# bfGraph/STGraph

Hardware: NVIDIA B200
Metric: gcn_fused_aggregation_fwd_bwd_algorithmic_hbm_gbs (higher is better)
Workload: dtype f32

## Files before the change

include/stgraph_b200.h:

```cpp
#ifndef STGRAPH_B200_H_
#define STGRAPH_B200_H_

#include <stddef.h>
#include <stdint.h>

#ifdef __cplusplus
extern "C" {
#endif

#define STG_ABI_VERSION 3

typedef enum StgStatus {
  STG_OK = 0,
  STG_ERR_INVALID_ARGUMENT = -1,
  STG_ERR_CUDA = -2,
  STG_ERR_UNSUPPORTED = -3,
  STG_ERR_WORKSPACE_TOO_SMALL = -4,
  STG_ERR_CAPACITY = -5
} StgStatus;

typedef struct StgCsrView {
  const int32_t* row_offset;
  const int32_t* column_indices;
  const int32_t* eids;
  const int32_t* node_ids;
  int32_t num_nodes;
  int32_t num_edges;
  int32_t eid_base;
  int32_t eids_identity;
  const int32_t* hub_rows;
  const int32_t* hub_count;
  int32_t hub_threshold;
  int32_t hub_capacity;
// ... 2 lines not shown

int stg_abi_version(void);
const char* stg_last_error(void);
int stg_device_info(int device, int32_t* sm_count, int64_t* l2_bytes, int32_t* cc_major, int32_t* cc_minor);

int stg_agg_scaled_sum_f32(const StgCsrView* g, const float* x, int32_t feat,
                           const float* nbr_scale, const float* edge_scale,
                           const float* row_scale, float* out, void* stream);

typedef struct StgEdgeMeta {
  int32_t col;
  float scale;
} StgEdgeMeta;

int stg_csr_pack_edge_meta_f32(const StgCsrView* g, const float* nbr_scale, const float* edge_scale,
                               StgEdgeMeta* meta, void* stream);

int stg_agg_packed_sum_f32(const StgCsrView* g, const StgEdgeMeta* meta, const float* x, int32_t feat,
                           const float* row_scale, float* out, int32_t accumulate, void* stream);

int stg_agg_packed_sum_strided_f32(const StgCsrView* g, const StgEdgeMeta* meta, const float* x, int32_t feat,
                                   int32_t x_ld, const float* row_scale, float* out, int32_t out_ld,
                                   int32_t accumulate, void* stream);

int stg_agg_scaled_sum_accum_f32(const StgCsrView* g, const float* x, int32_t feat, const float* nbr_scale,
                                 const float* edge_scale, const float* row_scale, float* out, void* stream);

int stg_agg_scaled_sum_red_f32(const StgCsrView* g, const float* x, int32_t feat, const float* nbr_scale,
                               const float* edge_scale, const float* row_scale, float* out, void* stream);

int stg_agg_scaled_sum_rows_f32(const StgCsrView* g, const int32_t* out_rows, const float* x, int32_t feat,
                                const float* nbr_scale, const float* edge_scale, const float* row_scale, float* out,
                                int32_t accumulate, void* stream);

int stg_agg_packed_sum_rows_f32(const StgCsrView* g, const StgEdgeMeta* meta, const int32_t* out_rows, const float* x,
                                int32_t feat, const float* row_scale, float* out, int32_t accumulate, void* stream);

#define STG_MAX_PARTS 16
int stg_agg_scaled_sum_parts_f32(const StgCsrView* g, const float* const* x_parts, const int32_t* part_bounds,
                                 int32_t num_parts, int32_t feat, const float* nbr_scale, const float* edge_scale,
                                 const float* row_scale, float* out, void* stream);

int stg_halo_pull_f32(const float* const* x_parts, const int32_t* part_bounds, int32_t num_parts, const int64_t* ids,
                      int64_t n_ids, int32_t feat, float* out, int32_t max_blocks, void* stream);

int stg_halo_push_f32(const float* own, int32_t feat, const int64_t* send_rows, const int32_t* send_peer,
// ... 147 lines not shown
```

stgraph_b200/_lib.py:

```python
from __future__ import annotations

import ctypes
import os
import subprocess
from ctypes import POINTER, Structure, c_char_p, c_float, c_int32, c_int64, c_size_t, c_void_p

_HERE = os.path.dirname(os.path.abspath(__file__))
LIB_PATH = os.environ.get("STG_B200_LIB") or os.path.join(_HERE, "lib", "libstgraph_b200.so")
CSRC_DIR = os.path.join(_HERE, "csrc")

ABI_VERSION = 3
VM_MAX_TENSORS = 24
VM_MAX_INSTR = 96
VM_MAX_REGS = 48
VM_MAX_ACC = 8


class StgCsrView(Structure):

    _fields_ = [
        ("row_offset", c_void_p),
        ("column_indices", c_void_p),
        ("eids", c_void_p),
        ("node_ids", c_void_p),
        ("num_nodes", c_int32),
        ("num_edges", c_int32),
        ("eid_base", c_int32),
        ("eids_identity", c_int32),
        ("hub_rows", c_void_p),
        ("hub_count", c_void_p),
        ("hub_threshold", c_int32),
        ("hub_capacity", c_int32),
        ("work_queue", c_void_p),
    ]


class StgVmTensor(Structure):
    _fields_ = [("side", c_int32), ("bc0", c_int32), ("bc1", c_int32), ("pad", c_int32)]


class StgVmInstr(Structure):
    _fields_ = [
        ("op", ctypes.c_int16),
        ("phase", ctypes.c_int16),
        ("dst", ctypes.c_int16),
        ("a", ctypes.c_int16),
        ("b", ctypes.c_int16),
        ("pad", ctypes.c_int16),
        ("imm", c_float),
    ]


class StgVmProgram(Structure):
    _fields_ = [
        ("dim0", c_int32),
        ("dim1", c_int32),
        ("n_tensors", c_int32),
        ("n_instr", c_int32),
        ("n_regs", c_int32),
        ("n_acc", c_int32),
        ("n_pre", c_int32),
        ("n_loop", c_int32),
        ("acc_init", c_float * VM_MAX_ACC),
        ("acc_kind", c_int32 * VM_MAX_ACC),
        ("tensors", StgVmTensor * VM_MAX_TENSORS),
        ("instr", StgVmInstr * VM_MAX_INSTR),
    ]


_P = POINTER
_SIGNATURES = {
    "stg_abi_version": (ctypes.c_int, [], False),
    "stg_last_error": (c_char_p, [], False),
    "stg_device_info": (ctypes.c_int, [ctypes.c_int, _P(c_int32), _P(c_int64), _P(c_int32), _P(c_int32)], True),
    "stg_agg_scaled_sum_f32": (ctypes.c_int, [_P(StgCsrView), c_void_p, c_int32, c_void_p, c_void_p, c_void_p,
                                              c_void_p, c_void_p], True),
    "stg_agg_scaled_sum_accum_f32": (ctypes.c_int, [_P(StgCsrView), c_void_p, c_int32, c_void_p, c_void_p, c_void_p,
                                                    c_void_p, c_void_p], True),
    "stg_agg_scaled_sum_red_f32": (ctypes.c_int, [_P(StgCsrView), c_void_p, c_int32, c_void_p, c_void_p, c_void_p,
                                                  c_void_p, c_void_p], True),
    "stg_agg_scaled_sum_rows_f32": (ctypes.c_int, [_P(StgCsrView), c_void_p, c_void_p, c_int32, c_void_p, c_void_p, c_void_p,
                                                   c_void_p, c_int32, c_void_p], True),
    "stg_csr_pack_edge_meta_f32": (ctypes.c_int, [_P(StgCsrView), c_void_p, c_void_p, c_void_p, c_void_p], True),
    "stg_agg_packed_sum_f32": (ctypes.c_int, [_P(StgCsrView), c_void_p, c_void_p, c_int32, c_void_p, c_void_p, c_int32,
                                              c_void_p], True),
    "stg_agg_packed_sum_strided_f32": (ctypes.c_int, [_P(StgCsrView), c_void_p, c_void_p, c_int32, c_int32, c_void_p,
                                                      c_void_p, c_int32, c_int32, c_void_p], True),
    "stg_halo_push_f32": (ctypes.c_int, [c_void_p, c_int32, c_void_p, c_void_p, c_void_p, c_int64, _P(c_void_p), c_int32,
                                         c_int32, c_void_p], True),
    "stg_agg_packed_sum_rows_f32": (ctypes.c_int, [_P(StgCsrView), c_void_p, c_void_p, c_void_p, c_int32, c_void_p,
                                                   c_void_p, c_int32, c_void_p], True),
    "stg_rows_gather_f32": (ctypes.c_int, [c_void_p, c_int32, c_void_p, c_int64, c_void_p, c_int32, c_void_p], True),
    "stg_halo_send_f32": (ctypes.c_int, [c_void_p, c_int32, c_int32, c_int32, _P(c_int64), _P(c_void_p), c_void_p], True),
    "stg_halo_exchange_f32": (ctypes.c_int, [c_void_p, c_int32, c_void_p, _P(c_int64), c_void_p, _P(c_void_p), _P(c_void_p),
                                              c_void_p, c_int32, c_int32, c_int32, c_int32, c_void_p], True),
    "stg_peer_signal": (ctypes.c_int, [_P(c_void_p), c_int32, c_int32, c_int32, c_void_p], True),
    "stg_peer_wait": (ctypes.c_int, [c_void_p, c_int32, c_int32, c_int32, c_int64, c_void_p, c_void_p], True),
    "stg_agg_scaled_sum_parts_f32": (ctypes.c_int, [_P(StgCsrView), _P(c_void_p), _P(c_int32), c_int32, c_int32, c_void_p,
                                                    c_void_p, c_void_p, c_void_p, c_void_p], True),
    "stg_halo_pull_f32": (ctypes.c_int, [_P(c_void_p), _P(c_int32), c_int32, c_void_p, c_int64, c_int32, c_void_p, c_int32,
                                         c_void_p], True),
    "stg_agg_scaled_sum_f32_host": (ctypes.c_int, [_P(StgCsrView), c_void_p, c_int32, c_void_p, c_void_p, c_void_p,
                                                   c_void_p, c_void_p, c_size_t, c_void_p], True),
    "stg_agg_scaled_sum_f32_host_async": (ctypes.c_int, [_P(StgCsrView), c_void_p, c_int32, c_void_p, c_void_p, c_void_p,
                                                         c_void_p, c_void_p, c_size_t, c_void_p], True),
# ... 91 lines not shown
```

stgraph_b200/csrc/agg.cu:

```cuda
#include "common.cuh"

#include <cooperative_groups.h>

#include <algorithm>
#include <cstdlib>

namespace stg {
namespace {

constexpr int kBlockThreads = 256;
constexpr int kHubThreads = 512;

template <int VEC>
__device__ __forceinline__ typename VecT<VEC>::type ld_row(const float* p) {
  using T = typename VecT<VEC>::type;
  return __ldg(reinterpret_cast<const T*>(p));
}
template <int VEC>
__device__ __forceinline__ void st_row(float* p, typename VecT<VEC>::type v) {
  using T = typename VecT<VEC>::type;
  __stcs(reinterpret_cast<T*>(p), v);
}

struct AggParams {
  const int32_t* __restrict__ row_off;
  const int32_t* __restrict__ col;
  const int32_t* __restrict__ eids;
  const int32_t* __restrict__ hub_rows;
  const int32_t* __restrict__ hub_count;
  const int32_t* __restrict__ out_rows;
  const int2* __restrict__ meta;
  int* queue;
  int num_rows;
  int num_edges;
  int eid_base;
  int eids_identity;
  int hub_threshold;
  int hub_capacity;
  const float* __restrict__ x;
  float* __restrict__ out;
  int ld;
  int ld_out;
  int width;
  const float* __restrict__ ns;
  const float* __restrict__ es;
  const float* __restrict__ rs;
  int accumulate;
  int nparts;
  int bounds[STG_MAX_PARTS + 1];
  const float* xs[STG_MAX_PARTS];
};

__device__ __forceinline__ void red_add(float* p, float v) { atomicAdd(p, v); }
__device__ __forceinline__ void red_add(float* p, float2 v) { atomicAdd(reinterpret_cast<float2*>(p), v); }
__device__ __forceinline__ void red_add(float* p, float4 v) { atomicAdd(reinterpret_cast<float4*>(p), v); }

__device__ __forceinline__ const float* src_row(const AggParams& p, int c) {
  int o = 0;
#pragma unroll
  for (int q = 1; q < STG_MAX_PARTS; ++q) o += (q < p.nparts && c >= p.bounds[q]) ? 1 : 0;
  return p.xs[o] + static_cast<size_t>(c - p.bounds[o]) * p.ld;
}

enum AggMode { kPlain = 0, kParts = 1, kPacked = 2 };

template <int MODE>
__device__ __forceinline__ void load_col(const AggParams& p, int base, int end, int gl, int& c, float& ms) {
  c = 0;
  ms = 0.f;
  const int e = base + gl;
  if (e < end) {
    if constexpr (MODE == kPacked) {
      const int2 m = __ldcs(p.meta + e);
// ... 278 lines not shown
}

template <int VEC, int GROUP, int NACC>
__device__ __forceinline__ void write_row(const AggParams& p, int row, int gl, bool nonempty, float r,
                                          typename VecT<VEC>::type (&acc)[NACC]) {
  typename VecT<VEC>::type none[NACC];
#pragma unroll
  for (int k = 0; k < NACC; ++k) zero_vec(none[k]);
  write_row<VEC, GROUP, NACC>(p, row, gl, nonempty, r, acc, false, none);
}

template <int VEC, int GROUP, int NACC>
__device__ __forceinline__ void prefetch_row(const AggParams& p, int row, int gl, typename VecT<VEC>::type (&old)[NACC]) {
  using T = typename VecT<VEC>::type;
  const float* dst = p.out + static_cast<size_t>(row) * p.ld_out;
#pragma unroll
  for (int k = 0; k < NACC; ++k) {
    const int o = (gl + k * GROUP) * VEC;
    zero_vec(old[k]);
    if (o < p.width) old[k] = *reinterpret_cast<const T*>(dst + o);
  }
}

template <int VEC, int GROUP, int NACC, int MINB, int UNROLL, int MODE, bool PAIR = false, bool GQ = false>
__global__ void __launch_bounds__(kBlockThreads, MINB) agg_rows_pipe_kernel(const AggParams p, int slots_per_block) {
  using T = typename VecT<VEC>::type;
  constexpr int GPW = 32 / GROUP;
  __shared__ int next_slot;
  const int lane = threadIdx.x & 31;
  const int gl = lane & (GROUP - 1);
  const int gidx = lane / GROUP;
  const unsigned gmask = (GROUP == 32) ? 0xffffffffu : (((1u << GROUP) - 1u) << (lane & ~(GROUP - 1)));
  const int total_slots = (p.num_rows + GPW - 1) / GPW;
  const int first = GQ ? 0 : blockIdx.x * slots_per_block;
  const int last = GQ ? total_slots : min(first + slots_per_block, total_slots);
  int q_cur = 0, q_pos = slots_per_block, q_nxt = 0;
  if constexpr (GQ) {
    if (lane == 0) q_nxt = atomicAdd(p.queue, 1);
  } else {
    if (threadIdx.x == 0) next_slot = first;
    __syncthreads();
  }

  auto draw = [&]() {
    if constexpr (GQ) {
      if (q_pos == slots_per_block && q_cur < total_slots) {
        q_cur = __shfl_sync(0xffffffffu, q_nxt, 0) * slots_per_block;
        q_pos = 0;
        if (lane == 0 && q_cur < total_slots) q_nxt = atomicAdd(p.queue, 1);
      }
      return q_cur + q_pos++;
    } else {
      int s = 0;
      if (lane == 0) s = atomicAdd(&next_slot, 1);
      return __shfl_sync(0xffffffffu, s, 0);
    }
  };
  auto finish = [&]() {
    if constexpr (GQ) {
      __syncthreads();
      if (threadIdx.x == 0 && atomicAdd(p.queue + 1, 1) == static_cast<int>(gridDim.x) - 1) {
        p.queue[0] = 0;
        p.queue[1] = 0;
        __threadfence();
      }
    }
    grid_dependency_wait();
  };
  auto stage_a = [&](int slot, int& row, int& beg, int& end) {
    row = slot * GPW + gidx;
    if (slot >= last || row >= p.num_rows) { row = 0; beg = 0; end = -1; return; }
    beg = __ldg(p.row_off + row);
    end = __ldg(p.row_off + row + 1);
    if (p.out_rows) row = __ldg(p.out_rows + row);
  };
  auto drop_hub = [&](int& beg, int& end) {
    if (p.hub_threshold > 0 && (end - beg) > p.hub_threshold) beg = 0, end = -1;
  };

  int slot0, row0, beg0, end0, c0;
  int row1, beg1, end1, c1;
  int row2, beg2, end2;
  float s0, r0, m0, m1;
  slot0 = draw();
  if (slot0 >= last) { finish(); return; }
  stage_a(slot0, row0, beg0, end0);
  int slot1 = draw();
  stage_a(slot1, row1, beg1, end1);
  int slot2 = draw();
  stage_a(slot2, row2, beg2, end2);
  drop_hub(beg0, end0);
  load_col<MODE>(p, beg0, end0, gl, c0, m0);
  drop_hub(beg1, end1);
  load_col<MODE>(p, beg1, end1, gl, c1, m1);
  load_scale<MODE>(p, beg0, end0, gl, c0, m0, s0);
  r0 = (end0 >= 0 && p.rs) ? __ldg(p.rs + row0) : 1.f;

  while (slot0 < last) {
    const int slot3 = draw();
    int row3, beg3, end3;
    stage_a(slot3, row3, beg3, end3);
    drop_hub(beg2, end2);
    int c2;
    float m2;
    load_col<MODE>(p, beg2, end2, gl, c2, m2);
    float s1;
    load_scale<MODE>(p, beg1, end1, gl, c1, m1, s1);
    const float r1 = (end1 >= 0 && p.rs) ? __ldg(p.rs + row1) : 1.f;

    if (end0 >= 0) {
      T acc[NACC];
      T old[NACC];
      const bool rmw = NACC <= 2 && p.accumulate == 1;
      if constexpr (NACC <= 2) {
        if (rmw) prefetch_row<VEC, GROUP, NACC>(p, row0, gl, old);
      }
      if constexpr (PAIR) {
        static_assert(VEC == 4 && GROUP == 32 && NACC == 1, "pair form: one row per warp, float4 lanes");
        accumulate_edges_pair<UNROLL, MODE>(p, beg0, end0, lane, acc[0], c0, 0.f, s0);
      } else {
#pragma unroll
        for (int k = 0; k < NACC; ++k) zero_vec(acc[k]);
        accumulate_edges<VEC, GROUP, NACC, UNROLL, MODE>(p, beg0, end0, 0, 1, gl, gmask, acc, c0, s0);
      }
      write_row<VEC, GROUP, NACC>(p, row0, gl, end0 > beg0, r0, acc, rmw, old);
    }
    slot0 = slot1; row0 = row1; beg0 = beg1; end0 = end1; c0 = c1; s0 = s1; r0 = r1;
    slot1 = slot2; row1 = row2; beg1 = beg2; end1 = end2; c1 = c2; m1 = m2;
    slot2 = slot3; row2 = row3; beg2 = beg3; end2 = end3;
  }
  finish();
}

template <int VEC, int GROUP, int NACC, int MODE, bool PAIR = false>
__global__ void __launch_bounds__(kBlockThreads) agg_rows_kernel(const AggParams p) {
  using T = typename VecT<VEC>::type;
  constexpr int GROUPS_PER_WARP = 32 / GROUP;
  const int lane = threadIdx.x & 31;
  const int gl = lane & (GROUP - 1);
  const unsigned gmask = (GROUP == 32) ? 0xffffffffu : (((1u << GROUP) - 1u) << (lane & ~(GROUP - 1)));
  const int warp = blockIdx.x * (kBlockThreads / 32) + (threadIdx.x >> 5);
  const int row = warp * GROUPS_PER_WARP + lane / GROUP;
  if (row >= p.num_rows) return;
  const int beg = __ldg(p.row_off + row);
  const int end = __ldg(p.row_off + row + 1);
  if (p.hub_threshold > 0 && (end - beg) > p.hub_threshold) return;

  T acc[NACC];
// ... 126 lines not shown
    return e == nullptr || e[0] != '0';
  }();
  return on;
}

inline int queue_chunk() {
  static const int v = [] {
    const char* e = getenv("STG_AGG_CHUNK");
    const int c = e ? atoi(e) : 4;
    return c < 0 ? 0 : (c > 4096 ? 4096 : c);
  }();
  return v;
}

inline int hub_grid_mult(int num_edges) {
  static const int v = [] {
    const char* e = getenv("STG_HUB_GRID");
    const int c = e ? atoi(e) : 0;
    return c < 0 ? 0 : (c > 4 ? 4 : c);
  }();
  return v > 0 ? v : (num_edges >= (1 << 24) ? 1 : 2);
}

template <int VEC, int GROUP, int NACC, int MODE>
int launch_agg(const AggParams& p, cudaStream_t stream) {
  constexpr int rows_per_block = (kBlockThreads / 32) * (32 / GROUP);
  const int blocks = (p.num_rows + rows_per_block - 1) / rows_per_block;
  const bool hubs = p.hub_threshold > 0 && p.hub_rows != nullptr;
  const bool overlap = hubs && p.num_edges >= (1 << 18);
  if (hubs) {
    agg_hub_kernel<VEC, GROUP, NACC, MODE><<<hub_grid_mult(p.num_edges) * (sm_count() / kHubCluster) * kHubCluster, kHubThreads, 0, stream>>>(p);
    STG_LAUNCH_CHECK("agg_hub_kernel");
  }
  if (blocks > 0) {
    const bool queue = p.num_rows >= 2 * sm_count() * 4 * (kBlockThreads / 32);
    bool launched = false;
    if constexpr (GROUP == 32 && MODE != kParts) if (queue) {
      launched = true;
      constexpr int MINB = 4;
      constexpr int kRowsPerWarp = 32;
      constexpr int slots_per_block = (kBlockThreads / 32) * kRowsPerWarp;
      const int pblocks = (p.num_rows + slots_per_block - 1) / slots_per_block;
      const bool gq = p.queue != nullptr && queue_chunk() > 0;
      const int gblocks = std::min(sm_count() * MINB, (p.num_rows + 7) / 8);
      if constexpr (VEC == 4 && NACC == 1) {
        if (p.width > 64 && pair_mode()) {
          if (gq) {
            STG_CUDA(launch_overlapped(agg_rows_pipe_kernel<VEC, GROUP, NACC, MINB, 8, MODE, true, true>, gblocks, kBlockThreads,
                                       stream, overlap, p, queue_chunk()));
          } else {
// ... 48 lines not shown
  return launch_agg<VEC, 32, 4, MODE>(p, stream);
}

__global__ void __launch_bounds__(256) pack_edge_meta_kernel(const AggParams p, int2* __restrict__ meta) {
  const int stride = gridDim.x * blockDim.x;
  for (int e = blockIdx.x * blockDim.x + threadIdx.x; e < p.num_edges; e += stride) {
    const int c = ld_stream(p.col + e);
    float sc = 1.f;
    if (p.ns) sc = __ldg(p.ns + c);
    if (p.es) {
      const int eid = p.eids_identity ? e : (ld_stream(p.eids + e) - p.eid_base);
      sc *= __ldg(p.es + eid);
    }
    __stcs(meta + e, make_int2(c, __float_as_int(sc)));
  }
}

}

int agg_scaled_sum_device(const StgCsrView* g, const float* x, int32_t feat, const float* ns,
                          const float* es, const float* rs, float* out, cudaStream_t stream,
                          int nparts = 0, const float* const* parts = nullptr, const int32_t* bounds = nullptr,
                          int accumulate = 0, const int32_t* out_rows = nullptr, const StgEdgeMeta* meta = nullptr,
                          int x_ld = 0, int out_ld = 0) {
  AggParams p;
  p.out_rows = out_rows;
  p.meta = reinterpret_cast<const int2*>(meta);
  p.queue = g->work_queue;
  p.accumulate = accumulate;
  p.nparts = nparts;
  for (int q = 0; q < STG_MAX_PARTS; ++q) p.xs[q] = q < nparts ? parts[q] : nullptr;
  for (int q = 0; q <= STG_MAX_PARTS; ++q) p.bounds[q] = (nparts > 0 && q <= nparts) ? bounds[q] : 0;
  p.row_off = g->row_offset;
  p.col = g->column_indices;
  p.eids = g->eids;
  p.hub_rows = g->hub_rows;
  p.hub_count = g->hub_count;
  p.num_rows = g->num_nodes;
  p.num_edges = g->num_edges;
  p.eid_base = g->eid_base;
  p.eids_identity = g->eids_identity;
  p.hub_threshold = (g->hub_rows && g->hub_count) ? g->hub_threshold : 0;
  p.hub_capacity = g->hub_capacity;
  p.ld = x_ld > 0 ? x_ld : feat;
  p.ld_out = out_ld > 0 ? out_ld : feat;
  p.ns = ns;
  p.es = es;
  p.rs = rs;
  bool al16 = aligned16(out), al8 = aligned8(out);
  if (nparts == 0) {
    al16 = al16 && aligned16(x);
    al8 = al8 && aligned8(x);
  }
  for (int q = 0; q < nparts; ++q) {
    al16 = al16 && aligned16(parts[q]);
    al8 = al8 && aligned8(parts[q]);
  }
  int vec = 1;
  if (feat % 4 == 0 && p.ld % 4 == 0 && p.ld_out % 4 == 0 && al16) vec = 4;
  else if (feat % 2 == 0 && p.ld % 2 == 0 && p.ld_out % 2 == 0 && al8) vec = 2;
  if (vec == 4 && feat > 32 && feat <= 64 && nparts == 0 && narrow_vec2() && g->work_queue != nullptr &&
      g->num_nodes >= 2 * sm_count() * 4 * (kBlockThreads / 32))
    vec = 2;
  const int chunk = 32 * 4 * vec;
  for (int f0 = 0; f0 < feat; f0 += chunk) {
    p.x = x ? x + f0 : nullptr;
    for (int q = 0; q < nparts; ++q) p.xs[q] = parts[q] + f0;
    p.out = out + f0;
    p.width = min(chunk, feat - f0);
    int rc;
    const int avg_degree = g->num_nodes > 0 ? g->num_edges / g->num_nodes : -1;
    if (nparts > 0) {
      if (vec == 4) rc = dispatch_group<4, kParts>(p, stream, avg_degree);
      else if (vec == 2) rc = dispatch_group<2, kParts>(p, stream, avg_degree);
      else rc = dispatch_group<1, kParts>(p, stream, avg_degree);
    } else if (meta != nullptr) {
      if (vec == 4) rc = dispatch_group<4, kPacked>(p, stream, avg_degree);
      else if (vec == 2) rc = dispatch_group<2, kPacked>(p, stream, avg_degree);
      else rc = dispatch_group<1, kPacked>(p, stream, avg_degree);
    } else {
      if (vec == 4) rc = dispatch_group<4, kPlain>(p, stream, avg_degree);
      else if (vec == 2) rc = dispatch_group<2, kPlain>(p, stream, avg_degree);
      else rc = dispatch_group<1, kPlain>(p, stream, avg_degree);
    }
    if (rc != STG_OK) return rc;
  }
  return STG_OK;
// ... 148 lines not shown
  const int blocks = static_cast<int>(std::min<int64_t>((static_cast<int64_t>(g->num_edges) + 255) / 256, 8 * sm_count()));
  pack_edge_meta_kernel<<<blocks, 256, 0, as_stream(stream)>>>(p, reinterpret_cast<int2*>(meta));
  STG_LAUNCH_CHECK("pack_edge_meta_kernel");
  return STG_OK;
}

STG_API int stg_agg_packed_sum_strided_f32(const StgCsrView* g, const StgEdgeMeta* meta, const float* x, int32_t feat,
                                           int32_t x_ld, const float* row_scale, float* out, int32_t out_ld,
                                           int32_t accumulate, void* stream) {
  int rc = validate_view(g, false);
  if (rc != STG_OK) return rc;
  STG_CHECK_ARG(feat > 0, "feat must be positive (got %d)", feat);
  STG_CHECK_ARG(x_ld >= feat && out_ld >= feat, "row strides (%d, %d) must be >= feat (%d)", x_ld, out_ld, feat);
  STG_CHECK_ARG(accumulate >= 0 && accumulate <= 2, "accumulate must be 0, 1 or 2 (got %d)", accumulate);
  if (g->num_nodes == 0) return STG_OK;
  STG_CHECK_ARG(g->num_edges == 0 || (meta != nullptr && aligned8(meta)),
                "meta must be a non-NULL, 8-byte aligned device pointer");
  STG_CHECK_ARG(x != nullptr && out != nullptr, "x / out is NULL");
  STG_CHECK_ARG(x != out, "x and out must not alias");
  return agg_scaled_sum_device(g, x, feat, nullptr, nullptr, row_scale, out, as_stream(stream), 0, nullptr, nullptr,
                               accumulate, nullptr, g->num_edges == 0 ? nullptr : meta, x_ld, out_ld);
}

STG_API int stg_agg_packed_sum_f32(const StgCsrView* g, const StgEdgeMeta* meta, const float* x, int32_t feat,
                                   const float* row_scale, float* out, int32_t accumulate, void* stream) {
  return stg_agg_packed_sum_strided_f32(g, meta, x, feat, feat, row_scale, out, feat, accumulate, stream);
}

STG_API int stg_agg_packed_sum_rows_f32(const StgCsrView* g, const StgEdgeMeta* meta, const int32_t* out_rows,
                                        const float* x, int32_t feat, const float* row_scale, float* out,
                                        int32_t accumulate, void* stream) {
  int rc = validate_view(g, false);
  if (rc != STG_OK) return rc;
  STG_CHECK_ARG(feat > 0, "feat must be positive (got %d)", feat);
  STG_CHECK_ARG(accumulate >= 0 && accumulate <= 2, "accumulate must be 0, 1 or 2 (got %d)", accumulate);
  if (g->num_nodes == 0) return STG_OK;
  STG_CHECK_ARG(g->num_edges == 0 || (meta != nullptr && aligned8(meta)),
                "meta must be a non-NULL, 8-byte aligned device pointer");
  STG_CHECK_ARG(x != nullptr && out != nullptr, "x / out is NULL");
  STG_CHECK_ARG(x != out, "x and out must not alias");
  return agg_scaled_sum_device(g, x, feat, nullptr, nullptr, row_scale, out, as_stream(stream), 0, nullptr, nullptr,
                               accumulate, out_rows, g->num_edges == 0 ? nullptr : meta);
}
```

stgraph_b200/graph/static/csr.py:

```python
from __future__ import annotations

import ctypes
import os

import numpy as np
import torch

from ... import _lib

HUB_THRESHOLD = int(os.environ.get("STG_HUB_THRESHOLD", "1024"))
PACK_META = os.environ.get("STG_PACK_META", "1") != "0"
MAX_META_REPACKS = 16


def _edges_to_device(edge_list, device, num_nodes=None):
    if isinstance(edge_list, tuple) and len(edge_list) == 2 and not np.isscalar(edge_list[0]) \
            and len(np.shape(edge_list[0])) == 1 and len(edge_list[0]) != 2:
        src, dst = edge_list
        src = torch.as_tensor(src)
        dst = torch.as_tensor(dst)
    else:
        if isinstance(edge_list, torch.Tensor):
            e = edge_list
        else:
            e = torch.from_numpy(np.asarray(edge_list, dtype=np.int64).reshape(-1, 2))
        e = e.reshape(-1, 2)
        src, dst = e[:, 0], e[:, 1]
    if src.is_floating_point() or dst.is_floating_point() or src.dtype == torch.bool:
        raise TypeError("vertex ids must be integers")
    src, dst = src.to(device=device), dst.to(device=device)
    if num_nodes is not None and src.numel() > 0:
        lo = int(torch.minimum(src.min(), dst.min()))
        hi = int(torch.maximum(src.max(), dst.max()))
        if lo < 0 or hi >= int(num_nodes):
# ... 72 lines not shown
            return None
        from ... import kernels

        meta = kernels.pack_edge_meta(self.view(), nbr_scale, edge_scale, device=self.row_offset.device)
        self._meta_cache = [(key, (nbr_scale, edge_scale), meta)] + self._meta_cache[:1]
        return meta

    def invalidate_packed_meta(self):
        if self._meta_misses > MAX_META_REPACKS:
            self.pack_enabled = bool(PACK_META)
        self._meta_cache = []
        self._meta_misses = 0

    def prepare_hub_schedule(self, sync: bool = True):
        n, e = self.num_nodes, self.num_edges
        cap = e // max(HUB_THRESHOLD, 1) + 1
        dev = self.row_offset.device
        self._hub_rows = torch.empty(cap, dtype=torch.int32, device=dev)
        self._hub_count = torch.zeros(1, dtype=torch.int32, device=dev)
        _lib.call("stg_csr_hub_rows", self.row_offset.data_ptr(), n, HUB_THRESHOLD, self._hub_rows.data_ptr(),
                  cap, self._hub_count.data_ptr(), _lib.current_stream_ptr())
        self._hub_enabled = True
        self._hub_sync = sync
        if sync:
            self._hub_enabled = int(self._hub_count.item()) > 0
        self._view = None
        self._alt_views = {}

    def view(self) -> _lib.StgCsrView:
        if self._view is None:
            v = _lib.StgCsrView()
            v.row_offset = self.row_offset.data_ptr()
            v.column_indices = self.column_indices.data_ptr()
            v.eids = self.eids.data_ptr() if self.eids is not None else None
            v.node_ids = self.node_ids.data_ptr() if self.node_ids is not None else None
            v.num_nodes = self.num_nodes
            v.num_edges = self.num_edges
            v.eid_base = self.eid_base
            v.eids_identity = 1 if self.eids_identity else 0
            if self._hub_enabled:
                v.hub_rows = self._hub_rows.data_ptr()
                v.hub_count = self._hub_count.data_ptr()
                v.hub_threshold = HUB_THRESHOLD
                v.hub_capacity = int(self._hub_rows.shape[0])
            else:
                v.hub_rows = None
                v.hub_count = None
                v.hub_threshold = 0
                v.hub_capacity = 0
            self._work_queue = torch.zeros(2, dtype=torch.int32, device=self.row_offset.device)
# ... 21 lines not shown
        enabled = True
        if getattr(self, "_hub_sync", False):
            cnt = min(int(count.item()), cap)
            enabled = cnt > 0
            if cnt > 1:
                r = rows[:cnt].long()
                length = (self.row_offset[r + 1] - self.row_offset[r]).long()
                order = torch.sort(length * self.num_nodes + (self.num_nodes - 1 - r), descending=True).indices
                rows[:cnt] = rows[:cnt][order]
        v = _lib.StgCsrView()
        for name, _ in _lib.StgCsrView._fields_:
            setattr(v, name, getattr(base, name))
        v.hub_rows = rows.data_ptr() if enabled else None
        v.hub_count = count.data_ptr() if enabled else None
        v.hub_threshold = threshold if enabled else 0
        v.hub_capacity = cap if enabled else 0
        alt[threshold] = (v, rows, count)
    return alt[threshold][0]


CSR.view_with_hub_threshold = _alt_view


def build_csr_pair(src: torch.Tensor, dst: torch.Tensor, num_nodes: int, want_perm: bool = False):
    assert src.is_cuda and dst.is_cuda, "stgraph_b200 builds graphs on the GPU only (no CPU fallback)"
    dev = src.device
    e = int(src.shape[0])
    n = int(num_nodes)
    i32 = dict(dtype=torch.int32, device=dev)
    f_ro = torch.empty(n + 1, **i32)
    f_col = torch.empty(e, **i32)
    f_eid = torch.empty(e, **i32)
    f_nid = torch.empty(n, **i32)
    b_ro = torch.empty(n + 1, **i32)
    b_col = torch.empty(e, **i32)
    b_eid = torch.empty(e, **i32)
    b_nid = torch.empty(n, **i32)
    in_deg = torch.empty(n, **i32)
    out_deg = torch.empty(n, **i32)
    perm = torch.empty(e, **i32) if want_perm else None
    n_unique = torch.zeros(1, **i32)
    ws_bytes = _lib.load().stg_csr_build_workspace_bytes(e, n)
    ws = torch.empty(ws_bytes, dtype=torch.uint8, device=dev)
    _lib.call("stg_csr_build", src.data_ptr(), dst.data_ptr(), e, n,
              f_ro.data_ptr(), f_col.data_ptr(), f_eid.data_ptr(), f_nid.data_ptr(),
              b_ro.data_ptr(), b_col.data_ptr(), b_eid.data_ptr(), b_nid.data_ptr(),
# ... 12 lines not shown
```

stgraph_b200/kernels.py:

```python
from __future__ import annotations

import ctypes

import torch

from . import _lib

launch_count = 0


def _check(t: torch.Tensor, name: str, dtype=torch.float32):
    if not isinstance(t, torch.Tensor):
        raise TypeError(f"{name} must be a torch.Tensor")
    if not t.is_cuda:
        raise RuntimeError(f"{name} must live on a CUDA device (stgraph_b200 has no CPU path)")
    if t.dtype != dtype:
        raise TypeError(f"{name} must be {dtype}, got {t.dtype}")
    if not t.is_contiguous():
        raise ValueError(f"{name} must be contiguous")
    return t


def agg_scaled_sum(view: _lib.StgCsrView, x: torch.Tensor, nbr_scale=None, edge_scale=None, row_scale=None,
                   out: torch.Tensor | None = None, accumulate=False, stream=None, out_rows=None) -> torch.Tensor:
    global launch_count
    _check(x, "x")
    n = view.num_nodes
    if out_rows is not None:
        _check(out_rows, "out_rows", torch.int32)
        if out is None or out_rows.numel() != n:
            raise ValueError("out_rows needs out= and one entry per view row")
        n = out.shape[0]
    if x.dim() < 2:
        raise ValueError("x must be [rows, feat...]")
    feat = x.numel() // max(x.shape[0], 1)
    for nm, t in (("nbr_scale", nbr_scale), ("edge_scale", edge_scale)):
        if t is not None:
            _check(t, nm)
    if nbr_scale is not None and nbr_scale.numel() != x.shape[0]:
        raise ValueError(f"nbr_scale must have one entry per row of x ({x.shape[0]}), got {nbr_scale.numel()}")
    if row_scale is not None:
        _check(row_scale, "row_scale")
        if row_scale.numel() != n:
            raise ValueError(f"row_scale must have {n} elements, got {row_scale.numel()}")
    if edge_scale is not None and edge_scale.numel() < view.num_edges:
        raise ValueError(f"edge_scale has {edge_scale.numel()} elements for {view.num_edges} edges")
    if out is None:
        if x.shape[0] != n:
            raise ValueError(f"x has {x.shape[0]} rows for a view of {n} rows: pass out= for a row slice")
        out = torch.empty_like(x)
    else:
        _check(out, "out")
        if out.shape[0] != n or out.numel() != n * feat:
            raise ValueError(f"out must be [{n}, {feat}], got {tuple(out.shape)}")
    if n == 0 or feat == 0 or view.num_nodes == 0:
        return out
    if out_rows is not None:
        _lib.call("stg_agg_scaled_sum_rows_f32", ctypes.byref(view), out_rows.data_ptr(), x.data_ptr(), feat,
                  _lib.ptr(nbr_scale), _lib.ptr(edge_scale), _lib.ptr(row_scale), out.data_ptr(),
                  {False: 0, True: 1, "red": 2}[accumulate], stream if stream is not None else _lib.current_stream_ptr())
        launch_count += 1 + (1 if view.hub_threshold > 0 else 0)
        return out
    fn = {False: "stg_agg_scaled_sum_f32", True: "stg_agg_scaled_sum_accum_f32", "red": "stg_agg_scaled_sum_red_f32"}[accumulate]
    _lib.call(fn, ctypes.byref(view), x.data_ptr(), feat, _lib.ptr(nbr_scale), _lib.ptr(edge_scale), _lib.ptr(row_scale),
              out.data_ptr(), stream if stream is not None else _lib.current_stream_ptr())
    launch_count += 1 + (1 if view.hub_threshold > 0 else 0)
    return out


def pack_edge_meta(view: _lib.StgCsrView, nbr_scale=None, edge_scale=None, out: torch.Tensor | None = None,
                   device=None) -> torch.Tensor:
    global launch_count
    for nm, t in (("nbr_scale", nbr_scale), ("edge_scale", edge_scale)):
        if t is not None:
            _check(t, nm)
    if edge_scale is not None and edge_scale.numel() < view.num_edges:
        raise ValueError(f"edge_scale has {edge_scale.numel()} elements for {view.num_edges} edges")
    if out is None:
        ref = nbr_scale if nbr_scale is not None else edge_scale
        dev = device if device is not None else (ref.device if ref is not None else torch.device("cuda", torch.cuda.current_device()))
        out = torch.empty(view.num_edges, 2, dtype=torch.int32, device=dev)
    else:
        _check(out, "out", torch.int32)
        if out.numel() != 2 * view.num_edges:
            raise ValueError(f"meta must be int32 [{view.num_edges}, 2]")
# ... 4 lines not shown
    launch_count += 1
    return out


def padded_rows(rows: int, feat: int, device, dtype=torch.float32) -> torch.Tensor:
    ld = (feat + 31) // 32 * 32
    return torch.empty(rows, ld, dtype=dtype, device=device)[:, :feat]


def _row_stride(t: torch.Tensor, name: str) -> int:
    if t.dim() == 2 and not t.is_contiguous():
        if not t.is_cuda:
            raise RuntimeError(f"{name} must live on a CUDA device (stgraph_b200 has no CPU path)")
        if t.dtype != torch.float32:
            raise TypeError(f"{name} must be torch.float32, got {t.dtype}")
        if t.shape[1] > 0 and (t.stride(1) != 1 or t.stride(0) < t.shape[1]):
            raise ValueError(f"{name} must have dense rows (stride(1) == 1, stride(0) >= feat)")
        return int(t.stride(0))
    _check(t, name)
    return t.numel() // max(t.shape[0], 1)


def agg_packed_sum(view: _lib.StgCsrView, meta: torch.Tensor, x: torch.Tensor, row_scale=None,
                   out: torch.Tensor | None = None, accumulate=False, stream=None) -> torch.Tensor:
    global launch_count
    x_ld = _row_stride(x, "x")
    _check(meta, "meta", torch.int32)
    n = view.num_nodes
    if meta.numel() < 2 * view.num_edges:
        raise ValueError(f"meta has {meta.numel() // 2} entries for {view.num_edges} edges")
    if x.dim() < 2:
        raise ValueError("x must be [rows, feat...]")
    feat = x.shape[1] if x.dim() == 2 else x.numel() // max(x.shape[0], 1)
    if row_scale is not None:
        _check(row_scale, "row_scale")
        if row_scale.numel() != n:
            raise ValueError(f"row_scale must have {n} elements, got {row_scale.numel()}")
    if out is None:
        if x.shape[0] != n:
            raise ValueError(f"x has {x.shape[0]} rows for a view of {n} rows: pass out= for a row slice")
        out = padded_rows(n, feat, x.device) if x_ld != feat else torch.empty_like(x)
    out_ld = _row_stride(out, "out")
    if out.shape[0] != n or out.numel() != n * feat:
        raise ValueError(f"out must be [{n}, {feat}], got {tuple(out.shape)}")
    if n == 0 or feat == 0:
        return out
    _lib.call("stg_agg_packed_sum_strided_f32", ctypes.byref(view), meta.data_ptr(), x.data_ptr(), feat, x_ld,
              _lib.ptr(row_scale), out.data_ptr(), out_ld, {False: 0, True: 1, "red": 2}[accumulate],
              stream if stream is not None else _lib.current_stream_ptr())
    launch_count += 1 + (1 if view.hub_threshold > 0 else 0)
    return out


def agg_packed_sum_rows(view: _lib.StgCsrView, meta: torch.Tensor, out_rows, x: torch.Tensor, row_scale, out: torch.Tensor,
                        accumulate=False, stream=None) -> torch.Tensor:
    global launch_count
    _check(x, "x")
    _check(out, "out")
    _check(meta, "meta", torch.int32)
    if meta.numel() < 2 * view.num_edges:
        raise ValueError(f"meta has {meta.numel() // 2} entries for {view.num_edges} edges")
    feat = x.numel() // max(x.shape[0], 1)
    if out.numel() != out.shape[0] * feat:
        raise ValueError(f"out must be [rows, {feat}], got {tuple(out.shape)}")
    if out_rows is not None:
        _check(out_rows, "out_rows", torch.int32)
        if out_rows.numel() != view.num_nodes:
            raise ValueError("out_rows needs one entry per view row")
    elif out.shape[0] != view.num_nodes:
        raise ValueError(f"out has {out.shape[0]} rows for a view of {view.num_nodes} rows")
    if row_scale is not None:
        _check(row_scale, "row_scale")
        if row_scale.numel() != out.shape[0]:
            raise ValueError(f"row_scale must have one entry per row of out ({out.shape[0]}), got {row_scale.numel()}")
    if view.num_nodes == 0 or feat == 0:
        return out
    _lib.call("stg_agg_packed_sum_rows_f32", ctypes.byref(view), meta.data_ptr(), _lib.ptr(out_rows), x.data_ptr(), feat,
              _lib.ptr(row_scale), out.data_ptr(), {False: 0, True: 1, "red": 2}[accumulate],
              stream if stream is not None else _lib.current_stream_ptr())
    launch_count += 1 + (1 if view.hub_threshold > 0 else 0)
    return out


def agg_scaled_sum_graph(csr, x: torch.Tensor, nbr_scale=None, edge_scale=None, row_scale=None,
                         out: torch.Tensor | None = None) -> torch.Tensor:
    meta = csr.packed_meta(nbr_scale, edge_scale) if getattr(csr, "pack_enabled", False) else None
    if meta is None:
        return agg_scaled_sum(csr.view(), x, nbr_scale, edge_scale, row_scale, out=out)
    return agg_packed_sum(csr.view(), meta, x, row_scale, out=out)


def gemm_tn(a: torch.Tensor, b: torch.Tensor, colsum: bool = False, out: torch.Tensor | None = None):
    global launch_count
    for nm, t in (("a", a), ("b", b)):
        if not t.is_cuda or t.dtype != torch.float32 or t.dim() != 2:
            raise TypeError(f"{nm} must be a 2-D float32 CUDA tensor")
        if t.shape[1] > 1 and t.stride(1) != 1:
            raise ValueError(f"{nm} must have unit stride along its rows (got strides {tuple(t.stride())})")
    if a.shape[0] != b.shape[0]:
        raise ValueError(f"a and b must have the same number of rows ({a.shape[0]} vs {b.shape[0]})")
    m, k, nc = a.shape[0], a.shape[1], b.shape[1]
    lda = a.stride(0) if m > 1 else max(k, 1)
    ldb = b.stride(0) if m > 1 else max(nc, 1)
    if out is not None and (out.shape != (k, nc) or not out.is_contiguous() or out.dtype != torch.float32):
        raise ValueError(f"out must be a contiguous float32 [{k}, {nc}] tensor")
    c = out if out is not None else torch.empty(k, nc, device=a.device, dtype=torch.float32)
    cs = torch.empty(nc, device=a.device, dtype=torch.float32) if colsum else None
    need = _lib.call("stg_gemm_tn_workspace_bytes", m, k, nc)
    ws = torch.empty(need // 4, device=a.device, dtype=torch.float32) if need else None
    _lib.call("stg_gemm_tn_f32", a.data_ptr(), lda, b.data_ptr(), ldb, m, k, nc, c.data_ptr(), _lib.ptr(cs), _lib.ptr(ws), need,
              _lib.current_stream_ptr())
    launch_count += 2 if need else 1
# ... 44 lines not shown
```

Before: 1003.

## Split hub rows into warp segments inside the persistent row-queue kernel

Adds a hub-segment schedule in which high-degree rows are split into 16 or 128 virtual slots interleaved with normal rows in one global work queue. Each warp accumulates its strided slice of edges into a partials buffer, and the last warp to finish, detected by an atomic counter, reduces the partials and writes the row. This folds the separate hub launch into a single kernel and balances load across warps. The cost is extra partial-buffer traffic, thread fences, and a host-side schedule built at graph setup.

Result: slower. 734.3, median of 6 (-26.8%).

```diff
diff --git a/include/stgraph_b200.h b/include/stgraph_b200.h
--- a/include/stgraph_b200.h
+++ b/include/stgraph_b200.h
@@ -8,7 +8,7 @@
 extern "C" {
 #endif
 
-#define STG_ABI_VERSION 3
+#define STG_ABI_VERSION 4
 
 typedef enum StgStatus {
   STG_OK = 0,
@@ -57,6 +57,23 @@
 int stg_agg_packed_sum_strided_f32(const StgCsrView* g, const StgEdgeMeta* meta, const float* x, int32_t feat,
                                    int32_t x_ld, const float* row_scale, float* out, int32_t out_ld,
                                    int32_t accumulate, void* stream);
+
+typedef struct StgHubSegments {
+  const int32_t* vslot;
+  const int32_t* segments;
+  int32_t* counters;
+  float* partials;
+  int64_t partial_capacity;
+  int32_t num_slots;
+  int32_t num_segments;
+} StgHubSegments;
+
+int stg_agg_scaled_sum_seg_f32(const StgCsrView* g, const StgHubSegments* seg, const float* x, int32_t feat,
+                               const float* nbr_scale, const float* edge_scale, const float* row_scale, float* out,
+                               void* stream);
+int stg_agg_packed_sum_seg_f32(const StgCsrView* g, const StgHubSegments* seg, const StgEdgeMeta* meta, const float* x,
+                               int32_t feat, int32_t x_ld, const float* row_scale, float* out, int32_t out_ld,
+                               void* stream);
 
 int stg_agg_scaled_sum_accum_f32(const StgCsrView* g, const float* x, int32_t feat, const float* nbr_scale,
                                  const float* edge_scale, const float* row_scale, float* out, void* stream);
diff --git a/stgraph_b200/_lib.py b/stgraph_b200/_lib.py
--- a/stgraph_b200/_lib.py
+++ b/stgraph_b200/_lib.py
@@ -9,7 +9,7 @@
 LIB_PATH = os.environ.get("STG_B200_LIB") or os.path.join(_HERE, "lib", "libstgraph_b200.so")
 CSRC_DIR = os.path.join(_HERE, "csrc")
 
-ABI_VERSION = 3
+ABI_VERSION = 4
 VM_MAX_TENSORS = 24
 VM_MAX_INSTR = 96
 VM_MAX_REGS = 48
@@ -35,6 +35,19 @@
     ]
 
 
+class StgHubSegments(Structure):
+
+    _fields_ = [
+        ("vslot", c_void_p),
+        ("segments", c_void_p),
+        ("counters", c_void_p),
+        ("partials", c_void_p),
+        ("partial_capacity", c_int64),
+        ("num_slots", c_int32),
+        ("num_segments", c_int32),
+    ]
+
+
 class StgVmTensor(Structure):
     _fields_ = [("side", c_int32), ("bc0", c_int32), ("bc1", c_int32), ("pad", c_int32)]
 
@@ -81,6 +94,10 @@
                                                   c_void_p, c_void_p], True),
     "stg_agg_scaled_sum_rows_f32": (ctypes.c_int, [_P(StgCsrView), c_void_p, c_void_p, c_int32, c_void_p, c_void_p, c_void_p,
                                                    c_void_p, c_int32, c_void_p], True),
+    "stg_agg_scaled_sum_seg_f32": (ctypes.c_int, [_P(StgCsrView), _P(StgHubSegments), c_void_p, c_int32, c_void_p, c_void_p,
+                                                  c_void_p, c_void_p, c_void_p], True),
+    "stg_agg_packed_sum_seg_f32": (ctypes.c_int, [_P(StgCsrView), _P(StgHubSegments), c_void_p, c_void_p, c_int32, c_int32,
+                                                  c_void_p, c_void_p, c_int32, c_void_p], True),
     "stg_csr_pack_edge_meta_f32": (ctypes.c_int, [_P(StgCsrView), c_void_p, c_void_p, c_void_p, c_void_p], True),
     "stg_agg_packed_sum_f32": (ctypes.c_int, [_P(StgCsrView), c_void_p, c_void_p, c_int32, c_void_p, c_void_p, c_int32,
                                               c_void_p], True),
diff --git a/stgraph_b200/csrc/agg.cu b/stgraph_b200/csrc/agg.cu
--- a/stgraph_b200/csrc/agg.cu
+++ b/stgraph_b200/csrc/agg.cu
@@ -10,6 +10,7 @@
 
 constexpr int kBlockThreads = 256;
 constexpr int kHubThreads = 512;
+constexpr int kHubWarps = kHubThreads / 32;
 
 template <int VEC>
 __device__ __forceinline__ typename VecT<VEC>::type ld_row(const float* p) {
@@ -49,6 +50,11 @@
   int nparts;
   int bounds[STG_MAX_PARTS + 1];
   const float* xs[STG_MAX_PARTS];
+  const int* __restrict__ vslot;
+  const int4* __restrict__ segs;
+  int* seg_count;
+  float* partials;
+  int vslots;
 };
 
 __device__ __forceinline__ void red_add(float* p, float v) { atomicAdd(p, v); }
@@ -373,16 +379,61 @@
   }
 }
 
-template <int VEC, int GROUP, int NACC, int MINB, int UNROLL, int MODE, bool PAIR = false, bool GQ = false>
-__global__ void __launch_bounds__(kBlockThreads, MINB) agg_rows_pipe_kernel(const AggParams p, int slots_per_block) {
+template <int VEC, int NACC, int MODE>
+__device__ __noinline__ void hub_segment(const AggParams& p, int seg, int lane) {
   using T = typename VecT<VEC>::type;
+  const int4 d = __ldg(p.segs + seg);
+  const int row = d.x, first = d.y, step = d.z;
+  const int beg = __ldg(p.row_off + row), end = __ldg(p.row_off + row + 1);
+  T acc[NACC];
+#pragma unroll
+  for (int k = 0; k < NACC; ++k) zero_vec(acc[k]);
+  accumulate_edges<VEC, 32, NACC, MODE>(p, beg, end, first, step, lane, 0xffffffffu, acc);
+  const int base = seg - first;
+#pragma unroll
+  for (int k = 0; k < NACC; ++k) {
+    const int o = (lane + k * 32) * VEC;
+    if (o < p.width) __stcg(reinterpret_cast<T*>(p.partials + static_cast<size_t>(seg) * p.width + o), acc[k]);
+  }
+  __threadfence();
+  __syncwarp();
+  int done = 0;
+  if (lane == 0) done = atomicAdd(p.seg_count + d.w, 1);
+  if (__shfl_sync(0xffffffffu, done, 0) != step - 1) return;
+  __threadfence();
+  T sum[NACC];
+#pragma unroll
+  for (int k = 0; k < NACC; ++k) {
+    const int o = (lane + k * 32) * VEC;
+    zero_vec(sum[k]);
+    if (o >= p.width) continue;
+    const T* q = reinterpret_cast<const T*>(p.partials + static_cast<size_t>(base) * p.width + o);
+    const size_t ld = static_cast<size_t>(p.width) / VEC;
+    for (int c = 0; c < step; c += kHubWarps) {
+      T cta = __ldcg(q + c * ld);
+      for (int w = 1; w < kHubWarps; ++w) add_vec(cta, __ldcg(q + (c + w) * ld));
+      if (c == 0) sum[k] = cta;
+      else add_vec(sum[k], cta);
+    }
+  }
+  const int orow = p.out_rows ? __ldg(p.out_rows + row) : row;
+  const float r = p.rs ? __ldg(p.rs + orow) : 1.f;
+  write_row<VEC, 32, NACC>(p, orow, lane, true, r, sum);
+  if (lane == 0) p.seg_count[d.w] = 0;
+}
+
+template <int VEC, int GROUP, int NACC, int MINB, int UNROLL, int MODE, bool PAIR = false, bool GQ = false, bool SEG = false>
+__global__ void __launch_bounds__(kBlockThreads, MINB) agg_rows_pipe_kernel(const __grid_constant__ AggParams p,
+                                                                             int slots_per_block) {
+  using T = typename VecT<VEC>::type;
+  static_assert(!SEG || (GQ && GROUP == 32), "hub segments: global queue, one row per warp");
   constexpr int GPW = 32 / GROUP;
   __shared__ int next_slot;
   const int lane = threadIdx.x & 31;
   const int gl = lane & (GROUP - 1);
   const int gidx = lane / GROUP;
   const unsigned gmask = (GROUP == 32) ? 0xffffffffu : (((1u << GROUP) - 1u) << (lane & ~(GROUP - 1)));
-  const int total_slots = (p.num_rows + GPW - 1) / GPW;
+  const int total_slots = SEG ? p.vslots : (p.num_rows + GPW - 1) / GPW;
   const int first = GQ ? 0 : blockIdx.x * slots_per_block;
   const int last = GQ ? total_slots : min(first + slots_per_block, total_slots);
   int q_cur = 0, q_pos = slots_per_block, q_nxt = 0;
@@ -418,7 +469,22 @@
     }
     grid_dependency_wait();
   };
+  auto stage_v = [&](int v, int& row, int& beg, int& end) {
+    row = v;
+    beg = 0;
+    end = -1;
+    if (v < 0) {
+      if (v != INT_MIN) end = v - 1;
+      return;
+    }
+    beg = __ldg(p.row_off + v);
+    end = __ldg(p.row_off + v + 1);
+  };
   auto stage_a = [&](int slot, int& row, int& beg, int& end) {
+    if constexpr (SEG) {
+      stage_v(slot < last ? __ldg(p.vslot + slot) : INT_MIN, row, beg, end);
+      return;
+    }
     row = slot * GPW + gidx;
     if (slot >= last || row >= p.num_rows) { row = 0; beg = 0; end = -1; return; }
     beg = __ldg(p.row_off + row);
@@ -433,9 +499,10 @@
   int row1, beg1, end1, c1;
   int row2, beg2, end2;
   float s0, r0, m0, m1;
+  auto more = [&](int slot, int end) { return SEG ? end != -1 : slot < last; };
   slot0 = draw();
-  if (slot0 >= last) { finish(); return; }
   stage_a(slot0, row0, beg0, end0);
+  if (!more(slot0, end0)) { finish(); return; }
   int slot1 = draw();
   stage_a(slot1, row1, beg1, end1);
   int slot2 = draw();
@@ -447,8 +514,8 @@
   load_scale<MODE>(p, beg0, end0, gl, c0, m0, s0);
   r0 = (end0 >= 0 && p.rs) ? __ldg(p.rs + row0) : 1.f;
 
-  while (slot0 < last) {
-    const int slot3 = draw();
+  while (more(slot0, end0)) {
+    int slot3 = draw();
     int row3, beg3, end3;
     stage_a(slot3, row3, beg3, end3);
     drop_hub(beg2, end2);
@@ -457,7 +524,7 @@
     load_col<MODE>(p, beg2, end2, gl, c2, m2);
     float s1;
     load_scale<MODE>(p, beg1, end1, gl, c1, m1, s1);
-    const float r1 = (end1 >= 0 && p.rs) ? __ldg(p.rs + row1) : 1.f;
+    float r1 = (end1 >= 0 && p.rs) ? __ldg(p.rs + row1) : 1.f;
 
     if (end0 >= 0) {
       T acc[NACC];
@@ -475,6 +542,15 @@
         accumulate_edges<VEC, GROUP, NACC, UNROLL, MODE>(p, beg0, end0, 0, 1, gl, gmask, acc, c0, s0);
       }
       write_row<VEC, GROUP, NACC>(p, row0, gl, end0 > beg0, r0, acc, rmw, old);
+    } else if (SEG && end0 < -1) {
+      hub_segment<VEC, NACC, MODE>(p, -(end0 + 2), lane);
+      stage_v(row1, row1, beg1, end1);
+      stage_v(row2, row2, beg2, end2);
+      stage_v(row3, row3, beg3, end3);
+      load_col<MODE>(p, beg1, end1, gl, c1, m1);
+      load_scale<MODE>(p, beg1, end1, gl, c1, m1, s1);
+      r1 = (end1 >= 0 && p.rs) ? __ldg(p.rs + row1) : 1.f;
+      load_col<MODE>(p, beg2, end2, gl, c2, m2);
     }
     slot0 = slot1; row0 = row1; beg0 = beg1; end0 = end1; c0 = c1; s0 = s1; r0 = r1;
     slot1 = slot2; row1 = row2; beg1 = beg2; end1 = end2; c1 = c2; m1 = m2;
@@ -647,10 +723,46 @@
   return v > 0 ? v : (num_edges >= (1 << 24) ? 1 : 2);
 }
 
+constexpr int kNotLaunched = 1;
+
+template <int VEC, int GROUP, int NACC, int MODE>
+int launch_agg_segments(const AggParams& p, cudaStream_t stream) {
+  if constexpr (GROUP == 32 && MODE != kParts) {
+    constexpr int MINB = 4;
+    const int chunk = queue_chunk();
+    if (p.vslot == nullptr || p.out_rows != nullptr || p.queue == nullptr || chunk <= 0 ||
+        p.num_rows < 2 * sm_count() * 4 * (kBlockThreads / 32))
+      return kNotLaunched;
+    AggParams q = p;
+    q.hub_threshold = 0;
+    const int gblocks = std::min(sm_count() * MINB, (p.num_rows + 7) / 8);
+    bool pair = false;
+    if constexpr (VEC == 4 && NACC == 1) {
+      if (p.width > 64 && pair_mode()) {
+        pair = true;
+        STG_CUDA(launch_overlapped(agg_rows_pipe_kernel<VEC, GROUP, NACC, MINB, 8, MODE, true, true, true>, gblocks,
+                                   kBlockThreads, stream, false, q, chunk));
+      }
+    }
+    if (!pair) {
+      STG_CUDA(launch_overlapped(agg_rows_pipe_kernel<VEC, GROUP, NACC, MINB, 8 / NACC, MODE, false, true, true>, gblocks,
+                                 kBlockThreads, stream, false, q, chunk));
+    }
+    STG_LAUNCH_CHECK("agg_rows_pipe_kernel (hub segments)");
+    return STG_OK;
+  } else {
+    (void)p;
+    (void)stream;
+    return kNotLaunched;
+  }
+}
+
 template <int VEC, int GROUP, int NACC, int MODE>
 int launch_agg(const AggParams& p, cudaStream_t stream) {
   constexpr int rows_per_block = (kBlockThreads / 32) * (32 / GROUP);
   const int blocks = (p.num_rows + rows_per_block - 1) / rows_per_block;
+  const int rc = launch_agg_segments<VEC, GROUP, NACC, MODE>(p, stream);
+  if (rc != kNotLaunched) return rc;
   const bool hubs = p.hub_threshold > 0 && p.hub_rows != nullptr;
   const bool overlap = hubs && p.num_edges >= (1 << 18);
   if (hubs) {
@@ -745,7 +857,7 @@
                           const float* es, const float* rs, float* out, cudaStream_t stream,
                           int nparts = 0, const float* const* parts = nullptr, const int32_t* bounds = nullptr,
                           int accumulate = 0, const int32_t* out_rows = nullptr, const StgEdgeMeta* meta = nullptr,
-                          int x_ld = 0, int out_ld = 0) {
+                          int x_ld = 0, int out_ld = 0, const StgHubSegments* seg = nullptr) {
   AggParams p;
   p.out_rows = out_rows;
   p.meta = reinterpret_cast<const int2*>(meta);
@@ -770,6 +882,11 @@
   p.ns = ns;
   p.es = es;
   p.rs = rs;
+  p.vslot = nullptr;
+  p.segs = nullptr;
+  p.seg_count = nullptr;
+  p.partials = nullptr;
+  p.vslots = 0;
   bool al16 = aligned16(out), al8 = aligned8(out);
   if (nparts == 0) {
     al16 = al16 && aligned16(x);
@@ -786,6 +903,14 @@
       g->num_nodes >= 2 * sm_count() * 4 * (kBlockThreads / 32))
     vec = 2;
   const int chunk = 32 * 4 * vec;
+  if (seg != nullptr && p.hub_threshold > 0 && nparts == 0 &&
+      static_cast<int64_t>(seg->num_segments) * std::min(chunk, static_cast<int>(feat)) <= seg->partial_capacity) {
+    p.vslot = seg->vslot;
+    p.segs = reinterpret_cast<const int4*>(seg->segments);
+    p.seg_count = seg->counters;
+    p.partials = seg->partials;
+    p.vslots = seg->num_slots;
+  }
   for (int f0 = 0; f0 < feat; f0 += chunk) {
     p.x = x ? x + f0 : nullptr;
     for (int q = 0; q < nparts; ++q) p.xs[q] = parts[q] + f0;
@@ -980,6 +1105,51 @@
                                accumulate, nullptr, g->num_edges == 0 ? nullptr : meta, x_ld, out_ld);
 }
 
+static int validate_segments(const StgHubSegments* seg) {
+  if (seg == nullptr) return STG_OK;
+  STG_CHECK_ARG(seg->num_slots >= 0 && seg->num_segments >= 0 && seg->partial_capacity >= 0,
+                "negative hub-segment sizes (%d slots, %d segments)", seg->num_slots, seg->num_segments);
+  STG_CHECK_ARG(seg->vslot != nullptr && seg->counters != nullptr, "hub segments: vslot / counters is NULL");
+  STG_CHECK_ARG(seg->num_segments == 0 || (seg->segments != nullptr && aligned16(seg->segments)),
+                "hub segments: the segment table must be a non-NULL, 16-byte aligned device pointer");
+  STG_CHECK_ARG(seg->partial_capacity == 0 || (seg->partials != nullptr && aligned16(seg->partials)),
+                "hub segments: partials must be a non-NULL, 16-byte aligned device pointer");
+  return STG_OK;
+}
+
+STG_API int stg_agg_scaled_sum_seg_f32(const StgCsrView* g, const StgHubSegments* seg, const float* x, int32_t feat,
+                                       const float* nbr_scale, const float* edge_scale, const float* row_scale, float* out,
+                                       void* stream) {
+  int rc = validate_view(g, edge_scale != nullptr);
+  if (rc != STG_OK) return rc;
+  rc = validate_segments(seg);
+  if (rc != STG_OK) return rc;
+  STG_CHECK_ARG(feat > 0, "feat must be positive (got %d)", feat);
+  if (g->num_nodes == 0) return STG_OK;
+  STG_CHECK_ARG(x != nullptr && out != nullptr, "x / out is NULL");
+  STG_CHECK_ARG(x != out, "x and out must not alias");
+  return agg_scaled_sum_device(g, x, feat, nbr_scale, edge_scale, row_scale, out, as_stream(stream), 0, nullptr, nullptr,
+                               0, nullptr, nullptr, 0, 0, seg);
+}
+
+STG_API int stg_agg_packed_sum_seg_f32(const StgCsrView* g, const StgHubSegments* seg, const StgEdgeMeta* meta,
+                                       const float* x, int32_t feat, int32_t x_ld, const float* row_scale, float* out,
+                                       int32_t out_ld, void* stream) {
+  int rc = validate_view(g, false);
+  if (rc != STG_OK) return rc;
+  rc = validate_segments(seg);
+  if (rc != STG_OK) return rc;
+  STG_CHECK_ARG(feat > 0, "feat must be positive (got %d)", feat);
+  STG_CHECK_ARG(x_ld >= feat && out_ld >= feat, "row strides (%d, %d) must be >= feat (%d)", x_ld, out_ld, feat);
+  if (g->num_nodes == 0) return STG_OK;
+  STG_CHECK_ARG(g->num_edges == 0 || (meta != nullptr && aligned8(meta)),
+                "meta must be a non-NULL, 8-byte aligned device pointer");
+  STG_CHECK_ARG(x != nullptr && out != nullptr, "x / out is NULL");
+  STG_CHECK_ARG(x != out, "x and out must not alias");
+  return agg_scaled_sum_device(g, x, feat, nullptr, nullptr, row_scale, out, as_stream(stream), 0, nullptr, nullptr, 0,
+                               nullptr, g->num_edges == 0 ? nullptr : meta, x_ld, out_ld, seg);
+}
+
 STG_API int stg_agg_packed_sum_f32(const StgCsrView* g, const StgEdgeMeta* meta, const float* x, int32_t feat,
                                    const float* row_scale, float* out, int32_t accumulate, void* stream) {
   return stg_agg_packed_sum_strided_f32(g, meta, x, feat, feat, row_scale, out, feat, accumulate, stream);
diff --git a/stgraph_b200/graph/static/csr.py b/stgraph_b200/graph/static/csr.py
--- a/stgraph_b200/graph/static/csr.py
+++ b/stgraph_b200/graph/static/csr.py
@@ -10,6 +10,10 @@
 
 HUB_THRESHOLD = int(os.environ.get("STG_HUB_THRESHOLD", "1024"))
 PACK_META = os.environ.get("STG_PACK_META", "1") != "0"
+HUB_SEGMENTS = os.environ.get("STG_HUB_SEGMENTS", "1") != "0"
+HUB_CTA_WARPS = 16
+HUB_CLUSTER_WARPS = 128
+CLUSTER_ROW_EDGES = 8192
 MAX_META_REPACKS = 16
 
 
@@ -128,10 +132,33 @@
                   cap, self._hub_count.data_ptr(), _lib.current_stream_ptr())
         self._hub_enabled = True
         self._hub_sync = sync
+        self._segments = None
         if sync:
             self._hub_enabled = int(self._hub_count.item()) > 0
+            if self._hub_enabled and HUB_SEGMENTS:
+                vslot, table, hubs = hub_segment_schedule(self.row_offset, HUB_THRESHOLD)
+                seg = _lib.StgHubSegments()
+                seg.vslot, seg.segments = vslot.data_ptr(), table.data_ptr()
+                counters = torch.zeros(hubs, dtype=torch.int32, device=dev)
+                seg.counters = counters.data_ptr()
+                seg.partials, seg.partial_capacity = None, 0
+                seg.num_slots, seg.num_segments = vslot.numel(), table.shape[0]
+                self._segments = (seg, vslot, table, counters, None)
         self._view = None
         self._alt_views = {}
+
+    def hub_segments(self, feat: int):
+        if getattr(self, "_segments", None) is None:
+            return None
+        seg, vslot, table, counters, partials = self._segments
+        need = seg.num_segments * min(int(feat), 512)
+        if need > seg.partial_capacity:
+            if torch.cuda.is_current_stream_capturing():
+                return None
+            partials = torch.empty(need, dtype=torch.float32, device=self.row_offset.device)
+            seg.partials, seg.partial_capacity = partials.data_ptr(), need
+            self._segments = (seg, vslot, table, counters, partials)
+        return seg
 
     def view(self) -> _lib.StgCsrView:
         if self._view is None:
@@ -199,6 +226,31 @@
 CSR.view_with_hub_threshold = _alt_view
 
 
+def hub_segment_schedule(row_offset: torch.Tensor, threshold: int):
+    ro = row_offset.long()
+    n = ro.numel() - 1
+    dev = row_offset.device
+    deg = ro[1:] - ro[:-1]
+    hub = deg > threshold
+    per_row = torch.ones(n, dtype=torch.long, device=dev)
+    per_row[hub] = torch.where(deg[hub] > CLUSTER_ROW_EDGES, HUB_CLUSTER_WARPS, HUB_CTA_WARPS)
+    slot_end = torch.cumsum(per_row, 0)
+    slot_beg = slot_end - per_row
+    hub_rows = hub.nonzero().squeeze(1)
+    k = per_row[hub_rows]
+    num_slots, nseg = int(slot_end[-1]) if n else 0, int(k.sum())
+    vslot = torch.empty(num_slots, dtype=torch.int32, device=dev)
+    rows = (~hub).nonzero().squeeze(1)
+    vslot[slot_beg[rows]] = rows.to(torch.int32)
+    seg_hub = torch.repeat_interleave(torch.arange(hub_rows.numel(), device=dev), k, output_size=nseg)
+    seg = torch.arange(nseg, device=dev)
+    first = seg - (torch.cumsum(k, 0) - k)[seg_hub]
+    seg_row = hub_rows[seg_hub]
+    vslot[slot_beg[seg_row] + first] = (-(seg + 1)).to(torch.int32)
+    segments = torch.stack([seg_row, first, k[seg_hub], seg_hub], 1).to(torch.int32).contiguous()
+    return vslot, segments, int(hub_rows.numel())
+
+
 def build_csr_pair(src: torch.Tensor, dst: torch.Tensor, num_nodes: int, want_perm: bool = False):
     assert src.is_cuda and dst.is_cuda, "stgraph_b200 builds graphs on the GPU only (no CPU fallback)"
     dev = src.device
diff --git a/stgraph_b200/kernels.py b/stgraph_b200/kernels.py
--- a/stgraph_b200/kernels.py
+++ b/stgraph_b200/kernels.py
@@ -22,7 +22,8 @@
 
 
 def agg_scaled_sum(view: _lib.StgCsrView, x: torch.Tensor, nbr_scale=None, edge_scale=None, row_scale=None,
-                   out: torch.Tensor | None = None, accumulate=False, stream=None, out_rows=None) -> torch.Tensor:
+                   out: torch.Tensor | None = None, accumulate=False, stream=None, out_rows=None,
+                   segments: _lib.StgHubSegments | None = None) -> torch.Tensor:
     global launch_count
     _check(x, "x")
     n = view.num_nodes
@@ -61,6 +62,14 @@
                   {False: 0, True: 1, "red": 2}[accumulate], stream if stream is not None else _lib.current_stream_ptr())
         launch_count += 1 + (1 if view.hub_threshold > 0 else 0)
         return out
+    if segments is not None:
+        if accumulate is not False or out_rows is not None:
+            raise ValueError("segments= takes the assigning form only")
+        _lib.call("stg_agg_scaled_sum_seg_f32", ctypes.byref(view), ctypes.byref(segments), x.data_ptr(), feat,
+                  _lib.ptr(nbr_scale), _lib.ptr(edge_scale), _lib.ptr(row_scale), out.data_ptr(),
+                  stream if stream is not None else _lib.current_stream_ptr())
+        launch_count += 1
+        return out
     fn = {False: "stg_agg_scaled_sum_f32", True: "stg_agg_scaled_sum_accum_f32", "red": "stg_agg_scaled_sum_red_f32"}[accumulate]
     _lib.call(fn, ctypes.byref(view), x.data_ptr(), feat, _lib.ptr(nbr_scale), _lib.ptr(edge_scale), _lib.ptr(row_scale),
               out.data_ptr(), stream if stream is not None else _lib.current_stream_ptr())
@@ -111,7 +120,8 @@
 
 
 def agg_packed_sum(view: _lib.StgCsrView, meta: torch.Tensor, x: torch.Tensor, row_scale=None,
-                   out: torch.Tensor | None = None, accumulate=False, stream=None) -> torch.Tensor:
+                   out: torch.Tensor | None = None, accumulate=False, stream=None,
+                   segments: _lib.StgHubSegments | None = None) -> torch.Tensor:
     global launch_count
     x_ld = _row_stride(x, "x")
     _check(meta, "meta", torch.int32)
@@ -134,6 +144,14 @@
         raise ValueError(f"out must be [{n}, {feat}], got {tuple(out.shape)}")
     if n == 0 or feat == 0:
         return out
+    if segments is not None:
+        if accumulate is not False:
+            raise ValueError("segments= takes the assigning form only")
+        _lib.call("stg_agg_packed_sum_seg_f32", ctypes.byref(view), ctypes.byref(segments), meta.data_ptr(), x.data_ptr(),
+                  feat, x_ld, _lib.ptr(row_scale), out.data_ptr(), out_ld,
+                  stream if stream is not None else _lib.current_stream_ptr())
+        launch_count += 1
+        return out
     _lib.call("stg_agg_packed_sum_strided_f32", ctypes.byref(view), meta.data_ptr(), x.data_ptr(), feat, x_ld,
               _lib.ptr(row_scale), out.data_ptr(), out_ld, {False: 0, True: 1, "red": 2}[accumulate],
               stream if stream is not None else _lib.current_stream_ptr())
@@ -174,9 +192,11 @@
 def agg_scaled_sum_graph(csr, x: torch.Tensor, nbr_scale=None, edge_scale=None, row_scale=None,
                          out: torch.Tensor | None = None) -> torch.Tensor:
     meta = csr.packed_meta(nbr_scale, edge_scale) if getattr(csr, "pack_enabled", False) else None
+    hub_segments = getattr(csr, "hub_segments", None)
+    seg = hub_segments(x.numel() // max(x.shape[0], 1)) if hub_segments is not None and x.dim() >= 2 else None
     if meta is None:
-        return agg_scaled_sum(csr.view(), x, nbr_scale, edge_scale, row_scale, out=out)
-    return agg_packed_sum(csr.view(), meta, x, row_scale, out=out)
+        return agg_scaled_sum(csr.view(), x, nbr_scale, edge_scale, row_scale, out=out, segments=seg)
+    return agg_packed_sum(csr.view(), meta, x, row_scale, out=out, segments=seg)
 
 
 def gemm_tn(a: torch.Tensor, b: torch.Tensor, colsum: bool = False, out: torch.Tensor | None = None):
```
